# kfirc1503/generative-audio

Measured on AMD Instinct MI355X. Metric: spectrogram-frames/sec, NPPC K=5 FullSubNet+ train step, higher is better.
Workload: dtype bf16

## Files before the change

generative-audio_amd/csrc/tcn.hip:

```cpp
#include <cstdlib>
#include "common.h"
#include "nppc_hip.h"

namespace {

enum { EPI_PLAIN = 0, EPI_PRELU_STATS = 1, EPI_RESIDUAL = 2, EPI_RELU = 3, EPI_PLAIN_F32 = 4, EPI_MASK_POS = 5, EPI_RESIDUAL_GN = 6 };

struct GemmArgs {
  const void* A; long lda; long strideA;
  const void* B; long ldb; long strideB;
  void* C; long ldc; long strideC;
  const float* bias; long strideBias;
  const void* res; long ldres; long strideRes;
  const float* slope; long strideSlope;
  double* stats; long strideStats;
  int R, N, K;
  int Tp, Tv;
  int Nv;
  int relu_in;
  int ksplit;
  const float* gnv; long strideGnv;
  double gcnt; float geps;
  int staged;
  float* colpart; long strideColpart;
// ... 1190 lines not shown
  dma_tile<DR_BM, BN, BR, STAGES>(A, lda, B, ldb, C + (size_t)bz * slab_stride, ldc, (long)bx * DR_BM, (long)by * BN, (long)by * BN,
                           rbase + (shift_a ? boff : 0), rbase + (shift_a ? 0 : boff), Rz, rs);
}

template <int BM, int BR, int STAGES>
__global__ __launch_bounds__(512, 1) void gemm_tn_dma2_kernel(const bf16_t* __restrict__ A, long lda, const bf16_t* __restrict__ B1,
                                                              long ldb1, int nt1, const bf16_t* __restrict__ B2, long ldb2, int N2,
                                                              float* __restrict__ C, long ldc, long slab_stride, long Rz,
                                                              float* __restrict__ rowsum) {
  unsigned bx = blockIdx.x, by = blockIdx.y, bz = blockIdx.z;
  dr_xcd_remap(bx, by, bz);
  const long m0 = (long)bx * BM, rbase = (long)bz * Rz;
  float* Cz = C + (size_t)bz * slab_stride;
  float* rs = rowsum != nullptr && by == 0 ? rowsum + (size_t)bz * ((size_t)gridDim.x * BM) : nullptr;
  if ((int)by >= nt1 && N2 == 64) {
    dma_tile<BM, 64, BR, STAGES>(A, lda, B2, ldb2, Cz, ldc, m0, 0, (long)nt1 * 192, rbase, rbase, Rz, nullptr);
    return;
  }
  const bool second = (int)by >= nt1;
  const long n0 = (long)(second ? by - nt1 : by) * 192;
  dma_tile<BM, 192, BR, STAGES>(A, lda, second ? B2 : B1, second ? ldb2 : ldb1, Cz, ldc, m0, n0, (long)by * 192, rbase, rbase, Rz, rs);
}

}

static bool tn_big_tiles() {
  static int v = -1;
  if (v < 0) {
    const char* e = getenv("NPPC_TN_BIG");
    v = (e && e[0] == '0') ? 0 : 1;
  }
  return v == 1;
}

static bool tn_dma() {
  static int v = -1;
  if (v < 0) {
    const char* e = getenv("NPPC_TN_DMA");
    v = (e && e[0] == '0') ? 0 : 1;
  }
  return v == 1;
}

static bool tn_dma192() {
  static int v = -1;
  if (v < 0) {
// ... 92 lines not shown
    return NPPC_OK;
  }
  if (M % DR_BM || (long)(M / DR_BM) * (nt1 + nt2) * ksplit < 256) return NPPC_EUNSUPPORTED;
  constexpr int smem = 5 * (32 * DR_BM * 2 + 32 * 192 * 2);
  static bool attr = false;
  if (!attr) {
    if (hipFuncSetAttribute(reinterpret_cast<const void*>(gemm_tn_dma2_kernel<DR_BM, 32, 5>),
                            hipFuncAttributeMaxDynamicSharedMemorySize, smem) != hipSuccess)
      return NPPC_ELAUNCH;
    attr = true;
  }
  hipLaunchKernelGGL((gemm_tn_dma2_kernel<DR_BM, 32, 5>), dim3(M / DR_BM, nt1 + nt2, ksplit), dim3(512), smem, s, (const bf16_t*)A,
                     lda, (const bf16_t*)B1, ldb1, nt1, (const bf16_t*)B2, ldb2, N2, C, ldc, (long)M * ldc, R / ksplit, rowsum);
  NPPC_CHECK_LAUNCH();
  return NPPC_OK;
}

extern "C" int nppc_gemm_tn_splitk_batched(const void* A, long lda, long sA, const void* B, long ldb, long sB, float* C, long ldc,
                                           long sC, int M, int N, long R, int ksplit, int batch, void* stream) {
  if (batch < 1) return NPPC_EBADARG;
  return launch_tn(A, lda, B, ldb, C, ldc, M, N, R, ksplit, 1, 0, 0, stream, batch, sA, sB, sC);
}

extern "C" int nppc_gemm_tn_splitk_taps(const void* A, long lda, const void* B, long ldb, float* C, long ldc, int M, int N,
                                        long R, int ksplit, int Wp, int shift_a, void* stream) {
  return launch_tn(A, lda, B, ldb, C, ldc, M, N, R, ksplit, 9, Wp, shift_a, stream);
}
```

generative-audio_amd/csrc/train_ops.hip:

```cpp
#include "common.h"
#include "nppc_hip.h"

namespace {

template <typename T>
__global__ __launch_bounds__(256) void transpose_kernel(const T* __restrict__ in, T* __restrict__ out, int rows, int cols,
                                                        long ld_in, long ld_out, long sIn, long sOut, int relu) {
  __shared__ float tile[32][33];
  in += (size_t)blockIdx.z * sIn;
  out += (size_t)blockIdx.z * sOut;
  const int r0 = blockIdx.x * 32, c0 = blockIdx.y * 32;
  const int tx = threadIdx.x & 31, ty = threadIdx.x >> 5;
  for (int i = ty; i < 32; i += 8) {
    const int r = r0 + i, c = c0 + tx;
    float v = 0.f;
    if (r < rows && c < cols) v = to_f32<T>(in[(size_t)r * ld_in + c]);
    if (relu) v = fmaxf(v, 0.f);
    tile[i][tx] = v;
  }
  __syncthreads();
  for (int i = ty; i < 32; i += 8) {
    const int c = c0 + i, r = r0 + tx;
    if (c < cols && r < rows) out[(size_t)c * ld_out + r] = from_f32<T>(tile[tx][i]);
  }
// ... 318 lines not shown
    float* d = dst + (size_t)rr * dst_ld + c;
    *d = accumulate ? *d + s : s;
  }
}

__global__ void reduce_slabs_t_kernel(const float* __restrict__ slabs, int S, long slab_stride, long ld, float* __restrict__ dst,
                                      long dst_ld, int rows, int ncols, long sSlab, long sDst) {
  slabs += (size_t)blockIdx.z * sSlab;
  dst += (size_t)blockIdx.z * sDst;
  __shared__ float tile[32][33];
  const int c0 = blockIdx.x * 32, r0 = blockIdx.y * 32;
  const int tx = threadIdx.x & 31, ty = threadIdx.x >> 5;
  for (int i = ty; i < 32; i += 8) {
    const int c = c0 + i, r = r0 + tx;
    float a = 0.f;
    if (c < ncols && r < rows)
      for (int s = 0; s < S; ++s) a += slabs[(size_t)s * slab_stride + (size_t)c * ld + r];
    tile[i][tx] = a;
  }
  __syncthreads();
  for (int i = ty; i < 32; i += 8) {
    const int r = r0 + i, c = c0 + tx;
    if (r < rows && c < ncols) dst[(size_t)r * dst_ld + c] = tile[tx][i];
  }
}

__global__ void adam_kernel(float* __restrict__ p, const float* __restrict__ g, float* __restrict__ m, float* __restrict__ v,
                            long n, float lr, float b1, float b2, float eps, float wd, float bc1, float bc2_sqrt,
                            float gscale, const double* __restrict__ sumsq, float max_norm,
                            const unsigned* const* __restrict__ guards = nullptr, int n_guards = 0, float* poison = nullptr) {
  for (int i = 0; i < n_guards; ++i)
    if (*guards[i] != 0u) {
      if (poison && blockIdx.x == 0 && threadIdx.x == 0) *poison = __builtin_nanf("");
      return;
    }
  if (sumsq) {
    const float total = (float)sqrt(sumsq[0]) * gscale;
    const float coef = max_norm / (total + 1e-6f);
    gscale *= coef < 1.f ? coef : 1.f;
  }
  for (long i = (long)blockIdx.x * blockDim.x + threadIdx.x; i < n; i += (long)gridDim.x * blockDim.x) {
    float gi = g[i] * gscale;
    const float pi = p[i];
    if (wd != 0.f) gi += wd * pi;
    const float mi = b1 * m[i] + (1.f - b1) * gi;
    const float vi = b2 * v[i] + (1.f - b2) * gi * gi;
// ... 167 lines not shown
  return NPPC_OK;
}

int nppc_reduce_slabs(const float* slabs, int S, long slab_stride, long ld, float* dst, long dst_ld, int rows, int col0,
                      int ncols, int permH, int accumulate, long sSlab, long sDst, int batch, void* stream) {
  if (!slabs || !dst || S < 1 || rows <= 0 || ncols <= 0) return NPPC_EBADARG;
  const long total = (long)rows * ncols;
  const int gx = (int)((total + 255) / 256 > 1024 ? 1024 : (total + 255) / 256);
  hipLaunchKernelGGL(reduce_slabs_kernel, dim3(gx, 1, batch), dim3(256), 0, (hipStream_t)stream, slabs, S, slab_stride, ld,
                     dst, dst_ld, rows, col0, ncols, permH, accumulate, sSlab, sDst);
  NPPC_CHECK_LAUNCH();
  return NPPC_OK;
}

int nppc_reduce_slabs_t(const float* slabs, int S, long slab_stride, long ld, float* dst, long dst_ld, int rows, int ncols,
                        long sSlab, long sDst, int batch, void* stream) {
  if (!slabs || !dst || S < 1 || rows <= 0 || ncols <= 0 || batch < 1) return NPPC_EBADARG;
  hipLaunchKernelGGL(reduce_slabs_t_kernel, dim3(ceil_div(ncols, 32), ceil_div(rows, 32), batch), dim3(256), 0,
                     (hipStream_t)stream, slabs, S, slab_stride, ld, dst, dst_ld, rows, ncols, sSlab, sDst);
  NPPC_CHECK_LAUNCH();
  return NPPC_OK;
}

int nppc_adam_step(float* p, const float* g, float* m, float* v, long n, double lr, double b1, double b2, double eps,
                   double wd, int step, double gscale, void* stream) {
  if (!p || !g || !m || !v || n <= 0 || step < 1) return NPPC_EBADARG;
  const double bc1 = 1.0 - pow(b1, (double)step);
  const double bc2s = sqrt(1.0 - pow(b2, (double)step));
  const int grid = (int)((n + 255) / 256 > 2048 ? 2048 : (n + 255) / 256);
  hipLaunchKernelGGL(adam_kernel, dim3(grid), dim3(256), 0, (hipStream_t)stream, p, g, m, v, n, (float)lr, (float)b1, (float)b2,
                     (float)eps, (float)wd, (float)bc1, (float)bc2s, (float)gscale, (const double*)nullptr, 0.f);
  NPPC_CHECK_LAUNCH();
  return NPPC_OK;
}

int nppc_adam_step_guarded(float* p, const float* g, float* m, float* v, long n, double lr, double b1, double b2, double eps,
                           double wd, int step, double gscale, const void* guards, int n_guards, float* poison, void* stream) {
  if (!p || !g || !m || !v || n <= 0 || step < 1 || n_guards < 0 || (n_guards > 0 && !guards)) return NPPC_EBADARG;
  const double bc1 = 1.0 - pow(b1, (double)step);
  const double bc2s = sqrt(1.0 - pow(b2, (double)step));
  const int grid = (int)((n + 255) / 256 > 2048 ? 2048 : (n + 255) / 256);
  hipLaunchKernelGGL(adam_kernel, dim3(grid), dim3(256), 0, (hipStream_t)stream, p, g, m, v, n, (float)lr, (float)b1, (float)b2,
                     (float)eps, (float)wd, (float)bc1, (float)bc2s, (float)gscale, (const double*)nullptr, 0.f,
                     (const unsigned* const*)guards, n_guards, poison);
  NPPC_CHECK_LAUNCH();
  return NPPC_OK;
// ... 16 lines not shown
```

generative-audio_amd/nppc_audio/_hip.py:

```python
import ctypes
import os

import torch

_HERE = os.path.dirname(os.path.abspath(__file__))
LIB_PATH = os.environ.get("NPPC_HIP_LIB") or os.path.join(_HERE, "libnppc_hip.so")

PREC_BF16 = 0
PREC_F32 = 1
_ERR = {1: "bad argument", 2: "kernel launch failed", 3: "unsupported shape/configuration"}

_lib = None

c_p = ctypes.c_void_p
c_i = ctypes.c_int
c_l = ctypes.c_long
c_f = ctypes.c_float


def lib():
    global _lib
    if _lib is None:
        if not os.path.exists(LIB_PATH):
            raise RuntimeError(
# ... 95 lines not shown
    "nppc_cirm_build_compress": [P, P, P, P, P, I, I, I, I, F, P],
    "nppc_cirm_decompress_apply_conj": [P, P, P, P, P, P, P, I, I, I, P],
    "nppc_cirm_decompress_apply": [P, P, P, P, P, P, P, I, I, I, P],
    "nppc_istft": [P, P, P, I, I, I, I, I, P],
    "nppc_rowsum": [P, P, L, I, P],
    "nppc_tsse_fwd": [P, P, P, P, P, P, P, P, I, I, I, P, P, P, P, P, P, P, P, P, P, P, P, I, I, I, I, P],
    "nppc_tsse_fwd_maps": [I, P, I, P, P, P, P, P, P, P, I, I, I, P, P, P, P, P, P, L, P, P, P, P, P, P, P, L, I, I, I, I, I, I, P],
    "nppc_tsse_bwd_maps": [I, P, L, P, I, P, P, P, P, I, I, I, P, P, P, L, P, P, P, P, P, P, P, P, P, P, P, P, P, P, P, P, P, P,
                           I, I, I, I, I, I, P],
    "nppc_scale_transpose": [I, P, P, P, I, I, I, I, I, I, P],
    "nppc_gemm_nt": [I, I, P, L, L, P, L, L, P, L, L, P, L, P, L, L, P, L, P, L, I, I, I, I, I, I, I, I, I, P],
    "nppc_tcn_mid_bwd_part_elems": [I, I, I, I, PL],
    "nppc_tcn_mid_bwd": [I, P, P, P, P, P, P, P, P, P, P, P, P, P, P, P, P, P, P, P, P, P, P, P, P, P, P, I, I, I, P,
                         I, I, I, I, I, F, L, L, L, I, I, P],
    "nppc_tcn_mid_bwd_finish": [P, L, P, L, I, I, I, P, P, P, P, P, P, P, P, P, P, I, I, L, L, I, I, P],
    "nppc_gemm_nt_colsum": [I, I, P, L, L, P, L, L, P, L, L, P, L, P, L, L, I, I, I, I, I, I, I, P, P],
    "nppc_gemm_nt_gn": [I, P, L, L, P, L, L, P, L, L, P, P, L, P, L, L, P, L, D, F, I, I, I, I, I, I, I, P],
    "nppc_tcn_pack_sconv": [I, P, P, P, P, P, P, P, I, I, I, I, I, I, L, L, L, L, P],
    "nppc_gemm_nt_splitk": [I, P, L, P, L, P, L, I, I, L, I, P],
    "nppc_gemm_tn_splitk": [P, L, P, L, P, L, I, I, L, I, P],
    "nppc_gemm_tn_splitk_rowsum": [P, L, P, L, P, L, I, I, L, I, P, P],
    "nppc_gemm_tn_splitk2": [P, L, P, L, I, P, L, I, P, L, I, L, I, P, P],
    "nppc_gemm_tn_splitk_batched": [P, L, L, P, L, L, P, L, L, I, I, L, I, I, P],
    "nppc_reduce_slabs_t": [P, I, L, L, P, L, I, I, L, L, I, P],
    "nppc_gemm_tn_splitk_taps": [P, L, P, L, P, L, I, I, L, I, I, I, P],
    "nppc_tcn_dwconv": [I, P, P, P, P, P, P, P, P, P, I, I, I, I, I, I, F, L, L, L, I, P],
    "nppc_tcn_gn_apply": [I, P, P, P, P, P, I, I, I, I, I, F, L, L, L, I, P],
    "nppc_pack_matrix": [I, P, P, I, I, I, I, I, P],
    "nppc_pack_matrix_batched": [I, P, P, I, I, I, I, I, I, I, L, L, L, L, P],
    "nppc_subband_mean": [I, P, I, P, I, L, P, P, P, I, I, I, I, I, P],
    "nppc_subband_stage": [I, P, I, P, I, L, P, P, I, I, I, I, I, I, I, I, P],
    "nppc_sb_head": [I, P, P, P, P, L, I, I, I, I, I, P],
    "nppc_gram": [P, P, P, P, P, I, I, L, P],
    "nppc_combine": [P, P, P, P, P, P, P, I, I, L, P],
    "nppc_gs_solve": [P, P, P, I, I, I, P],
    "nppc_gs_bwd_solve": [P, P, P, P, I, I, I, P],
    "nppc_loss_solve": [P, P, P, P, P, P, P, P, P, P, I, I, P],
    "nppc_loss_bwd_coef": [P, P, P, F, F, P, I, I, P],
    "nppc_loss_bwd_coef_dev": [P, P, P, P, F, F, P, I, I, P],
    "nppc_transpose": [I, P, P, I, I, L, L, L, L, I, I, P],
    "nppc_colsum": [I, P, P, I, I, L, L, L, I, P, L, P],
    "nppc_colsum_scratch_elems": [I, I, I, PL],
    "nppc_sb_head_bwd": [I, P, P, P, P, P, P, L, I, I, I, I, I, P],
    "nppc_subband_stage_bwd": [I, P, P, P, P, P, P, I, I, I, I, I, L, I, I, I, P],
    "nppc_subband_unfold_bwd": [I, P, P, P, P, P, I, I, I, I, I, I, I, I, P],
    "nppc_reduce_slabs": [P, I, L, L, P, L, I, I, I, I, I, L, L, I, P],
# ... 146 lines not shown
```

generative-audio_amd/nppc_audio/engine.py:

```python
import ctypes
import os

import numpy as np
import torch

from . import _hip as H
from .ops_lstm import (PackedLSTM, PackedLSTMBwd, ROW_PAD, WGRAD_SPLITS, bwd_head_fusable, forward_x_ld, lstm2_backward, lstm2_forward,
                       own_workspaces, padded_rows,
                       rows_view, workspace)

TCN_HIDDEN = 512
TCN_DILATIONS = (1, 2, 5, 9, 1, 2, 5, 9)
BRANCHES = ("", "_real", "_imag")
EPI_PLAIN, EPI_PRELU_STATS, EPI_RESIDUAL, EPI_RELU, EPI_PLAIN_F32, EPI_MASK_POS = 0, 1, 2, 3, 4, 5


def rup(a, b):
    return (a + b - 1) // b * b


TCN_WGRAD_ON_SIDE = os.environ.get("NPPC_TCN_WGRAD_SIDE", "1") != "0"
TCN_WGRAD_SPLITS = int(os.environ.get("NPPC_TCN_S2", "8"))
FC_WGRAD_AT_END = os.environ.get("NPPC_FC_AT_END", "1") != "0"
TCN_WGRAD_MAIN_BLOCKS = int(os.environ.get("NPPC_TCN_WGRAD_MAIN_BLOCKS", "1"))
MID_FINISH_DEFER = os.environ.get("NPPC_MID_FINISH_DEFER", "1") != "0"
COLSUM_IN_GEMM = os.environ.get("NPPC_COLSUM_IN_GEMM", "1") != "0"
TN_PAIRED = os.environ.get("NPPC_TN_PAIRED", "1") != "0"
FUSED_HEAD = int(os.environ.get("NPPC_FUSED_HEAD", "3"))


class FlatParams:

    def __init__(self, module, device):
        named = list(module.named_parameters())
        total = sum(p.numel() for _, p in named)
        self.flat = torch.empty(total, dtype=torch.float32, device=device)
        self.grad = None
        self.off = {}
        o = 0
        for n, p in named:
            k = p.numel()
            self.flat[o:o + k].copy_(p.detach().reshape(-1))
            p.data = self.flat[o:o + k].view(p.shape)
            self.off[n] = (o, tuple(p.shape))
            o += k
        self.named = named

    def view(self, name):
        o, shp = self.off[name]
# ... 49 lines not shown

class FSNEngine:
    import weakref as _weakref
    _unjoined = _weakref.WeakValueDictionary()

    def __init__(self, flat, *, num_freqs, n_maps, out_size, sb_neighbors, look_ahead, sb_hidden, groups, kersize,
                 prec, trainable):
        self.fp = flat
        self.F, self.nm, self.O = num_freqs, n_maps, out_size
        self.nb, self.la, self.Hd, self.G = sb_neighbors, look_ahead, sb_hidden, groups
        self.ks = tuple(kersize)
        self.prec = prec
        self.dt = H.dtype_of(prec)
        self.trainable = trainable
        self.C = n_maps * num_freqs
        self.ldC = rup(self.C, 64)
        self.ldF = rup(num_freqs, 64)
        self.KC = self.ldC
        self.dev = flat.flat.device
        self.I = 2 * sb_neighbors + 1 + 3
        self.sP = flat.branch_stride()
        self.sAtt = flat.attention_stride()
        self.packed_version = None
        self._side = None
        self._gen = 0
        self.last_train = None
        self.grad_range_hook = None
        self.early_buckets_ok = self._check_bucket_layout() if trainable else False
        self.pre_lstm_hook = None
        self.defer_join = False
        self.join_pending = False
        self.bufs = {}
        own_workspaces(self)
        self.lstm = PackedLSTM(self.I, self.Hd, prec, self.dev)
        self.KX = self.lstm.kx
        self.mult = torch.from_numpy(unfold_multiplicity(self.F, self.nb)).to(self.dev)
        C, ldC, ldF = self.C, self.ldC, self.ldF
        self.W1p = torch.zeros(8, 3, TCN_HIDDEN, ldC, dtype=self.dt, device=self.dev)
        self.W2p = torch.zeros(8, 3, ldC, TCN_HIDDEN, dtype=self.dt, device=self.dev)
        self.u2 = torch.zeros(8, 3, ldC, dtype=torch.float32, device=self.dev)
        self.v2 = torch.zeros(8, 3, ldC, dtype=torch.float32, device=self.dev)
        self.Wfcp = torch.zeros(3, ldF, ldC, dtype=self.dt, device=self.dev)
        self.Opad = rup(self.O, 16)
        self.Whp = torch.zeros(self.Opad, self.Hd, dtype=self.dt, device=self.dev)
        if trainable:
            if self.O > 32:
# ... 403 lines not shown
            with torch.cuda.stream(self._side):
                self._side.wait_event(ev)
                fn()

        def fc_wgrad(slab):
            q = H.stream()
            H.colsum(prec, dpre_fb, self.g("fb_model.fc_output_layer.bias"), R, F, ldF, R * ldF, sP, 3,
                     lambda n: ws("cs_fc", (n,), torch.float32), q)
            H.call("nppc_transpose", prec, dpre_fb, tA, R, F, ldF, R, R * ldF, sTA, 0, 3, q)
            H.call("nppc_transpose", prec, X8, tB, R, ldC, ldC, R, R * ldC, sTB, 1, 3, q)
            self._wgrad(tA, R, sTA, tB, R, sTB, Fr, ldC, R, S2, "fb_model.fc_output_layer.weight", C, F, C, slab, batch=3, sDst=sP)
        fc_ok = prec == H.PREC_BF16 and TCN_HIDDEN % 128 == 0 and ldC % 64 == 0 and R % (64 * S2) == 0
        fc_at_end = fc_ok and FC_WGRAD_AT_END
        if fc_ok and not fc_at_end:
            on_side(lambda: fc_wgrad(slab2))
        elif not fc_ok:
            fc_wgrad(slab2)
        tn_ok = prec == H.PREC_BF16 and TCN_HIDDEN % 128 == 0 and ldC % 64 == 0 and R % (64 * S2) == 0
        if tn_ok:
            dXL = [ws(f"dX_{i}", (3, B, Tp, ldC)) for i in range(9)]
            a2L = [ws(f"a2_{i}", (3, B, Tp, TCN_HIDDEN), zero=True) for i in range(8)]
            h2L = [ws(f"h2b_{i}", (3, B, Tp, TCN_HIDDEN)) for i in range(8)]
            dXa, dXb = dXL[8], dXL[7]
        else:
            dXa = ws("dXa", (3, B, Tp, ldC))
            dXb = ws("dXb", (3, B, Tp, ldC))

        bk = 64 if prec == H.PREC_BF16 else 32
        cs_ok = tn_ok and COLSUM_IN_GEMM and ldF % bk == 0 and TCN_HIDDEN % bk == 0
        cp_all = ws("colpart", (8, 3, R // 128, ldC), torch.float32) if cs_ok else None
        cpL = [cp_all[i] for i in range(8)] if cs_ok else None
        if cs_ok:
            H.call("nppc_gemm_nt_colsum", prec, EPI_MASK_POS, dpre_fb, ldF, R * ldF, self.WfcT, ldF, ldC * ldF, dXa, ldC, R * ldC,
                   None, 0, X8, ldC, R * ldC, R, ldC, ldF, Tp, Tv, C, 3, cpL[7], s)
        else:
            H.call("nppc_gemm_nt", prec, EPI_MASK_POS, dpre_fb, ldF, R * ldF, self.WfcT, ldF, ldC * ldF, dXa, ldC, R * ldC, None, 0,
                   X8, ldC, R * ldC, None, 0, None, 0, R, ldC, ldF, Tp, Tv, C, 0, 3, 1, s)
        sAct = B * Tp * TCN_HIDDEN
        h1b = ws("h1b", (3, B, Tp, TCN_HIDDEN))
        h2b = ws("h2b", (3, B, Tp, TCN_HIDDEN))
        Smid = ws("Smid", (3, B, TCN_HIDDEN // 64, 8), torch.float64)
        n_part = H.mid_bwd_part_elems(B, TCN_HIDDEN, Tp, 3)
        Pmid = ws("Pmid", (8, n_part), torch.float32)
        lay = self.fp.off["fb_model.sequence_model.1.conv1x1.weight"][0] - self.fp.off["fb_model.sequence_model.0.conv1x1.weight"][0]

        def finish_mid(lo, hi):
            pre_ = f"fb_model.sequence_model.{lo}."
            H.call("nppc_tcn_mid_bwd_finish", Pmid[lo], n_part, cpL[lo] if cs_ok else None, 3 * (R // 128) * ldC, R // 128, ldC, C,
                   self.g(pre_ + "norm2.weight"), self.g(pre_ + "norm2.bias"), self.g(pre_ + "norm1.weight"), self.g(pre_ + "norm1.bias"),
                   self.g(pre_ + "depthwise_conv.weight"), self.g(pre_ + "depthwise_conv.bias"), self.g(pre_ + "prelu1.weight"),
                   self.g(pre_ + "prelu2.weight"), self.g(pre_ + "conv1x1.bias"), self.g(pre_ + "sconv.bias") if cs_ok else None,
                   B, TCN_HIDDEN, sP, lay, 3, hi - lo, s)
        early = self.grad_range_hook is not None and self.early_buckets_ok
        defer_finish = MID_FINISH_DEFER
        dXo, dXi = dXa, dXb
        for i in range(7, -1, -1):
            pre = f"fb_model.sequence_model.{i}."
            dil = TCN_DILATIONS[i]
            st1, st2 = d["stats"][i, 0], d["stats"][i, 1]
            y1, y2, Xin = d["y1"][i], d["y2"][i], d["X"][i]
            if tn_ok:
                dXo, dXi, a2, h2b = dXL[i + 1], dXL[i], a2L[i], h2L[i]
            else:
                a2 = d["a2"]
            if not cs_ok:
                H.colsum(prec, dXo, self.g(pre + "sconv.bias"), R, C, ldC, R * ldC, sP, 3,
                         lambda n: ws("cs_sconv", (n,), torch.float32), s)
            H.call("nppc_gemm_nt", prec, EPI_PLAIN, dXo, ldC, R * ldC, self.W2T[i], ldC, TCN_HIDDEN * ldC, h1b, TCN_HIDDEN,
                   sAct, None, 0, None, 0, 0, None, 0, None, 0, R, TCN_HIDDEN, ldC, Tp, Tv, TCN_HIDDEN, 0, 3, 1, s)
            H.call("nppc_tcn_mid_bwd", prec, h1b, y2, y1, st1, st2, Smid, Pmid[i], self.p(pre + "norm1.weight"), self.p(pre + "norm1.bias"),
                   self.p(pre + "norm2.weight"), self.p(pre + "norm2.bias"), self.p(pre + "depthwise_conv.weight"),
                   self.p(pre + "prelu1.weight"), self.p(pre + "prelu2.weight"), a2, h2b, self.g(pre + "norm2.weight"),
                   self.g(pre + "norm2.bias"), self.g(pre + "norm1.weight"), self.g(pre + "norm1.bias"),
                   self.g(pre + "depthwise_conv.weight"), self.g(pre + "depthwise_conv.bias"), self.g(pre + "prelu1.weight"),
                   self.g(pre + "prelu2.weight"), self.g(pre + "conv1x1.bias"),
                   cpL[i] if cs_ok else None, R // 128, ldC, C, self.g(pre + "sconv.bias") if cs_ok else None,
                   B, TCN_HIDDEN, Tp, Tv, dil, 1e-8, sAct, B * 2, sP, 3, 0 if defer_finish else 1, s)
            if i == 4 and early and defer_finish:
                finish_mid(4, 8)
            if tn_ok:
                inline = i < TCN_WGRAD_MAIN_BLOCKS
                wslab = ws("slab_main", (3 * S2 * TCN_HIDDEN * ldC,), torch.float32) if inline else slab2

                def sconv_wgrad(a2=a2, dXo=dXo, dest=self.g(pre + "sconv.weight"), wslab=wslab):
                    q = H.stream()
                    H.call("nppc_gemm_tn_splitk_batched", a2, TCN_HIDDEN, sAct, dXo, ldC, R * ldC, wslab, ldC,
                           S2 * TCN_HIDDEN * ldC, TCN_HIDDEN, ldC, R, S2, 3, q)
                    H.call("nppc_reduce_slabs_t", wslab, S2, TCN_HIDDEN * ldC, ldC, dest, TCN_HIDDEN, C, TCN_HIDDEN,
                           S2 * TCN_HIDDEN * ldC, sP, 3, q)
                if inline:
                    sconv_wgrad()
                else:
                    on_side(sconv_wgrad)
            else:
                H.call("nppc_transpose", prec, dXo, tA, R, ldC, ldC, R, R * ldC, sTA, 0, 3, s)
                H.call("nppc_transpose", prec, a2, tB, R, TCN_HIDDEN, TCN_HIDDEN, R, sAct, sTB, 0, 3, s)
                self._wgrad(tA, R, sTA, tB, R, sTB, Cr, TCN_HIDDEN, R, S2, pre + "sconv.weight", TCN_HIDDEN, C, TCN_HIDDEN,
                            slab2, batch=3, sDst=sP)
            if tn_ok:
                def c1_wgrad(h2b=h2b, Xin=Xin, dest=self.g(pre + "conv1x1.weight"), wslab=wslab):
                    q = H.stream()
                    H.call("nppc_gemm_tn_splitk_batched", h2b, TCN_HIDDEN, sAct, Xin, ldC, R * ldC, wslab, ldC,
                           S2 * TCN_HIDDEN * ldC, TCN_HIDDEN, ldC, R, S2, 3, q)
                    H.call("nppc_reduce_slabs", wslab, S2, TCN_HIDDEN * ldC, ldC, dest, C, TCN_HIDDEN, 0, C, 0, 0,
                           S2 * TCN_HIDDEN * ldC, sP, 3, q)
                if inline:
                    c1_wgrad()
                else:
                    on_side(c1_wgrad)
            else:
                H.call("nppc_transpose", prec, h2b, tA, R, TCN_HIDDEN, TCN_HIDDEN, R, sAct, sTA, 0, 3, s)
                H.call("nppc_transpose", prec, Xin, tB, R, ldC, ldC, R, R * ldC, sTB, 0, 3, s)
                self._wgrad(tA, R, sTA, tB, R, sTB, TCN_HIDDEN, ldC, R, S2, pre + "conv1x1.weight", C, TCN_HIDDEN, C, slab2,
                            batch=3, sDst=sP)
            if cs_ok and i > 0:
                H.call("nppc_gemm_nt_colsum", prec, EPI_RESIDUAL, h2b, TCN_HIDDEN, sAct, self.W1T[i], TCN_HIDDEN, ldC * TCN_HIDDEN,
                       dXi, ldC, R * ldC, None, 0, dXo, ldC, R * ldC, R, ldC, TCN_HIDDEN, Tp, Tv, C, 3, cpL[i - 1], s)
            else:
                H.call("nppc_gemm_nt", prec, EPI_RESIDUAL, h2b, TCN_HIDDEN, sAct, self.W1T[i], TCN_HIDDEN, ldC * TCN_HIDDEN, dXi, ldC,
                       R * ldC, None, 0, dXo, ldC, R * ldC, None, 0, None, 0, R, ldC, TCN_HIDDEN, Tp, Tv, C, 0, 3, 1, s)
            dXo, dXi = dXi, dXo
            if i == 4 and self.grad_range_hook is not None and self.early_buckets_ok:
# ... 60 lines not shown
```

include/nppc_hip.h:

```cpp
#ifndef NPPC_HIP_H
#define NPPC_HIP_H
#ifdef __cplusplus
extern "C" {
#endif

int nppc_stft(const float* wave, float* re, float* im, float* mag , int B, int L, int nfft, int hop,
              void* stream);
int nppc_dropband(const float* in, float* out, int B, int C, int F, int T, int G, void* stream);
int nppc_cirm_build_compress(const float* nr, const float* ni, const float* cr, const float* ci, float* out, int B, int F,
                             int T, int G, float eps, void* stream);
int nppc_cirm_decompress_apply_conj(const float* crm, const float* nr, const float* ni, float* dec ,
                                    float* emag, float* ere, float* eim, int B, int F, int T, void* stream);

int nppc_cirm_decompress_apply(const float* crm, const float* nr, const float* ni, float* dec , float* emag,
                               float* ere, float* eim, int B, int F, int T, void* stream);
int nppc_istft(const float* re, const float* im, float* out, int B, int T, int nfft, int hop, int L, void* stream);

int nppc_rowsum(const float* x, double* sums, long R, int T, void* stream);
int nppc_tsse_fwd_maps(int prec, const float* const* maps, int nmaps, double* rowsum, const float* cw0, const float* cb0,
                       const float* cw1, const float* cb1, const float* cw2, const float* cb2, int ks0, int ks1, int ks2,
                       const float* fcw, const float* fcb, const float* w1, const float* b1, const float* w2, const float* b2, long sW,
                       float* scale, float* ns, float* pre, float* sq, float* h1, float* sg, void* X0, long sY, int B, int C, int T,
                       int look_ahead, int Tp, int ld, void* stream);
int nppc_tsse_bwd_ws_elems(int nmaps, int B, int C, int ks0, int ks1, int ks2, long* elems);
// ... 11 lines not shown
int nppc_tsse_bwd(int prec, const void* dX0, const float* x, const double* rowsum, const float* cw0, const float* cw1,
                  const float* cw2, int ks0, int ks1, int ks2, const float* fcw, const float* w1, const float* w2,
                  const float* ns, const float* pre, const float* sq, const float* h1, const float* sg, float* dsg_ws,
                  float* g_cw0, float* g_cb0, float* g_cw1, float* g_cb1, float* g_cw2, float* g_cb2, float* g_fcw,
                  float* g_fcb, float* g_w1, float* g_b1, float* g_w2, float* g_b2, int B, int C, int T, int look_ahead, int Tp,
                  int ld, int coff, void* stream);
int nppc_scale_transpose(int prec, const float* x, const float* scale , void* y, int B, int C, int T, int Tp,
                         int ld, int coff, void* stream);

int nppc_gemm_nt(int prec, int epi, const void* A, long lda, long sA, const void* B, long ldb, long sB, void* C, long ldc,
                 long sC, const float* bias, long sBias, const void* res, long ldres, long sRes, const float* slope,
                 long sSlope, double* stats, long sStats, int R, int N, int K, int Tp, int Tv, int Nv, int relu_in,
                 int batch, int ksplit, void* stream);
int nppc_gemm_nt_splitk(int prec, const void* A, long lda, const void* B, long ldb, float* C, long ldc, int M, int N, long K,
                        int ksplit, void* stream);
int nppc_gemm_tn_splitk(const void* A, long lda, const void* B, long ldb, float* C, long ldc, int M, int N, long R, int ksplit,
                        void* stream);
int nppc_gemm_tn_splitk_rowsum(const void* A, long lda, const void* B, long ldb, float* C, long ldc, int M, int N, long R,
                               int ksplit, float* rowsum, void* stream);
int nppc_gemm_tn_splitk2(const void* A, long lda, const void* B1, long ldb1, int N1, const void* B2, long ldb2, int N2, float* C,
                         long ldc, int M, long R, int ksplit, float* rowsum, void* stream);
int nppc_gemm_tn_splitk_batched(const void* A, long lda, long sA, const void* B, long ldb, long sB, float* C, long ldc, long sC,
                                int M, int N, long R, int ksplit, int batch, void* stream);
int nppc_gemm_tn_splitk_taps(const void* A, long lda, const void* B, long ldb, float* C, long ldc, int M, int N, long R,
                             int ksplit, int Wp, int shift_a, void* stream);
int nppc_pack_matrix(int prec, const float* src, void* dst, int N, int K, int Npad, int ldd, int transpose, void* stream);
int nppc_pack_matrix_batched(int prec, const float* src, void* dst, int N, int K, int Npad, int ldd, int transpose, int n_a,
                             int n_b, long src_stride_a, long src_stride_b, long dst_stride_a, long dst_stride_b, void* stream);
int nppc_tcn_dwconv(int prec, const void* in, void* out, const double* st1, double* st2, const float* gamma,
                    const float* beta, const float* wd, const float* bd, const float* slope2, int B, int Cc, int ld, int Tp,
                    int Tv, int dil, float eps, long sAct, long sSt, long sP, int batch, void* stream);
int nppc_tcn_gn_apply(int prec, const void* in, void* out, const double* st, const float* gamma, const float* beta, int B,
                      int Cc, int ld, int Tp, int Tv, float eps, long sAct, long sSt, long sP, int batch, void* stream);
int nppc_tcn_gn_bwd(int prec, const void* dA, const void* y, const double* st, const float* gamma, const float* slope,
                    double* S, void* dpre, float* dgamma, float* dbeta, float* dslope, int B, int Cc, int Tp, int Tv, float eps,
                    long sAct, long sSt, long sP, int batch, void* stream);
int nppc_tcn_dwconv_bwd(int prec, const void* du, const void* y1, const double* st1, const float* gamma, const float* beta,
                        const float* wd, void* dz, float* dwd, float* dbd, int B, int Cc, int Tp, int Tv, int dil, float eps,
                        long sAct, long sSt, long sP, int batch, void* stream);
int nppc_tcn_mid_bwd_part_elems(int B, int Cc, int Tp, int batch, long* n);
int nppc_tcn_mid_bwd(int prec, const void* dA, const void* y2, const void* y1, const double* st1, const double* st2, double* S,
                     float* part,
                     const float* gamma1, const float* beta1, const float* gamma2, const float* beta2, const float* wd,
                     const float* slope1, const float* slope2, void* a2, void* dpre1, float* dgamma2, float* dbeta2,
                     float* dgamma1, float* dbeta1, float* dwd, float* dbd, float* dslope1, float* dslope2, float* dbias1,
                     const float* colpart, int cp_tiles, int cp_ld, int cp_cols, float* dbias2, int B,
                     int Cc, int Tp, int Tv, int dil, float eps, long sAct, long sSt, long sP, int batch, int finish_now,
                     void* stream);
int nppc_tcn_mid_bwd_finish(const float* part, long partL, const float* colpart, long colpartL, int cp_tiles, int cp_ld,
                            int cp_cols, float* dgamma2, float* dbeta2, float* dgamma1, float* dbeta1, float* dwd, float* dbd,
                            float* dslope1, float* dslope2, float* dbias1, float* dbias2, int B, int Cc, long sP, long sL,
                            int batch, int nblk, void* stream);
int nppc_gemm_nt_gn(int prec, const void* A, long lda, long sA, const void* Wg, long ldb, long sB, void* C, long ldc, long sC,
                    const float* u, const float* v, long sUV, const void* res, long ldres, long sRes, const double* stats,
                    long sStats, double cnt, float eps, int R, int N, int K, int Tp, int Tv, int Nv, int batch, void* stream);
int nppc_gemm_nt_colsum(int prec, int epi, const void* A, long lda, long sA, const void* B, long ldb, long sB, void* C, long ldc,
                        long sC, const float* bias, long sBias, const void* res, long ldres, long sRes, int R, int N, int K,
                        int Tp, int Tv, int Nv, int batch, float* colpart, void* stream);
int nppc_tcn_pack_sconv(int prec, const float* W, const float* gamma, const float* beta, const float* bias, void* Wg, float* u,
                        float* v, int N, int K, int Npad, int ldd, int n_a, int n_b, long src_stride_a, long src_stride_b,
                        long dst_stride_a, long dst_stride_b, void* stream);
int nppc_transpose(int prec, const void* in, void* out, int rows, int cols, long ld_in, long ld_out, long sIn, long sOut,
                   int relu, int batch, void* stream);
int nppc_colsum_scratch_elems(int rows, int cols, int batch, long* n);
int nppc_colsum(int prec, const void* M, float* out, int rows, int cols, long ld, long sM, long sOut, int batch,
                float* scratch, long scratch_elems, void* stream);
int nppc_reduce_slabs_t(const float* slabs, int S, long slab_stride, long ld, float* dst, long dst_ld, int rows, int ncols,
                        long sSlab, long sDst, int batch, void* stream);
int nppc_reduce_slabs(const float* slabs, int S, long slab_stride, long ld, float* dst, long dst_ld, int rows, int col0,
                      int ncols, int permH, int accumulate, long sSlab, long sDst, int batch, void* stream);

int nppc_subband_mean(int prec, const void* src, int ldS, const void* fb, int ldF, long strideFb, const float* mult,
                      float* scale, double* work, int B, int F, int Tp, int Tv, int nfeat, void* stream);
int nppc_subband_stage(int prec, const void* src, int ldS, const void* fb, int ldF, long strideFb, const float* scale,
                       void* x, int B, int F, int Tp, int Tv, int nb, int G, int KX, int ones_col, void* stream);
int nppc_subband_stage_bwd(int prec, const void* dx, const void* x, const void* fb, const float* scale, double* D,
                           void* dpre, int B, int F, int Tp, int Tv, int ldF, long strideFb, int nb, int G, int KX,
                           void* stream);
int nppc_subband_unfold_bwd(int prec, const void* dx, const float* scale, const double* D, const float* mult, void* dX0,
                            int ldX, int B, int F, int Tp, int Tv, int nb, int G, int KX, void* stream);
int nppc_sb_head(int prec, const void* h2, const void* wh, const float* bias, float* out, long Nseq, int Tn, int la,
                 int Hd, int O, int Fo, void* stream);
int nppc_sb_head_bwd(int prec, const float* dout, const void* whT, const void* h2, void* dh2, float* dWh, float* dbh,
                     long Nseq, int Tn, int la, int Hd, int O, int Fo, void* stream);

int nppc_lstm2_packed_elems(int I, int H, long* n1, long* n2, int* kx);
int nppc_lstm2_pack_weights(int prec, const float* w_ih0, const float* w_hh0, const float* b_ih0, const float* b_hh0,
                            const float* w_ih1, const float* w_hh1, const float* b_ih1, const float* b_hh1, int I, int H,
                            void* wp1, void* wp2, float* bias1, float* bias2, void* stream);
int nppc_lstm2_fwd(int prec, int train, int mtile, const void* x, const void* wp1, const void* wp2, const float* bias1,
                   const float* bias2, void* h2, void* h1, void* g1, void* g2, void* c1, void* c2, long N, int Tn, int I,
// ... 336 lines not shown
```

Before: 254,900.

## Group TCN weight-gradient GEMMs across blocks into single grouped split-K launches

Adds a grouped TN split-K GEMM kernel that takes per-problem pointer tables, plus a grouped slab-reduction kernel that vectorises reads and can write either transposed or plain output. The engine accumulates the sconv and conv1x1 weight-gradient GEMMs of several TCN blocks and issues them as one grouped GEMM and one grouped reduce on the side stream. This replaces many small per-block launches and separate transposes, which should cut launch overhead and improve GPU fill. In exchange, gradients become available later for the groups, and the pointer tables are cached per set of data pointers.

```diff
diff --git a/generative-audio_amd/csrc/tcn.hip b/generative-audio_amd/csrc/tcn.hip
--- a/generative-audio_amd/csrc/tcn.hip
+++ b/generative-audio_amd/csrc/tcn.hip
@@ -1236,6 +1236,36 @@
   dma_tile<BM, 192, BR, STAGES>(A, lda, second ? B2 : B1, second ? ldb2 : ldb1, Cz, ldc, m0, n0, (long)by * 192, rbase, rbase, Rz, rs);
 }
 
+constexpr int TN_GROUP_MAX = 48;
+struct TnGroup {
+  const bf16_t* A[TN_GROUP_MAX];
+  const bf16_t* B[TN_GROUP_MAX];
+  float* C[TN_GROUP_MAX];
+  int lda[TN_GROUP_MAX], ldb[TN_GROUP_MAX], ldc[TN_GROUP_MAX];
+};
+
+__device__ __forceinline__ void dr_xcd_remap_any(unsigned& bx, unsigned& by, unsigned& bz) {
+  const unsigned tiles = gridDim.x * gridDim.y;
+  const unsigned lin = bx + gridDim.x * (by + gridDim.y * bz);
+  if (lin < tiles * (gridDim.z & ~7u)) {
+    const unsigned xcd = lin & 7, j = lin >> 3;
+    bz = xcd + 8 * (j / tiles);
+    const unsigned t = j % tiles;
+    bx = t % gridDim.x;
+    by = t / gridDim.x;
+  }
+}
+
+template <int BN, int BR, int STAGES>
+__global__ __launch_bounds__(512, 1) void gemm_tn_dma_grouped_kernel(const TnGroup g, int M, long Rz, int ksplit) {
+  unsigned bx = blockIdx.x, by = blockIdx.y, bz = blockIdx.z;
+  dr_xcd_remap_any(bx, by, bz);
+  const unsigned p = bz / (unsigned)ksplit, z = bz % (unsigned)ksplit;
+  const long ldc = g.ldc[p];
+  dma_tile<DR_BM, BN, BR, STAGES>(g.A[p], g.lda[p], g.B[p], g.ldb[p], g.C[p] + (size_t)z * M * ldc, ldc, (long)bx * DR_BM,
+                                  (long)by * BN, (long)by * BN, (long)z * Rz, (long)z * Rz, Rz, nullptr);
+}
+
 }
 
 static bool tn_big_tiles() {
@@ -1374,6 +1404,57 @@
   return launch_tn(A, lda, B, ldb, C, ldc, M, N, R, ksplit, 1, 0, 0, stream, batch, sA, sB, sC);
 }
 
+extern "C" int nppc_gemm_tn_grouped(const void* const* A, const long* lda, const void* const* B, const long* ldb, float* const* C,
+                                    const long* ldc, int M, int N, long R, int ksplit, int P, void* stream) {
+  if (!A || !lda || !B || !ldb || !C || !ldc || M <= 0 || N <= 0 || R <= 0 || ksplit < 1 || P < 1) return NPPC_EBADARG;
+  if (P > TN_GROUP_MAX || (long)P * ksplit > 65535 || !tn_dma() || M % DR_BM || R % ksplit) return NPPC_EUNSUPPORTED;
+  const int bn = N % 192 == 0 ? 192 : (N % 128 == 0 ? 128 : 0);
+  const long Rz = R / ksplit;
+  if (bn == 0 || Rz % (bn == 192 ? 32 : 64)) return NPPC_EUNSUPPORTED;
+  TnGroup g;
+  for (int p = 0; p < P; ++p) {
+    if (!A[p] || !B[p] || !C[p] || lda[p] < M || ldb[p] < N || ldc[p] < N || lda[p] % 8 || ldb[p] % 8) return NPPC_EBADARG;
+    if (lda[p] > 0x7fffffffL || ldb[p] > 0x7fffffffL || ldc[p] > 0x7fffffffL) return NPPC_EBADARG;
+    if (((size_t)A[p] | (size_t)B[p]) & 15) return NPPC_EBADARG;
+    g.A[p] = (const bf16_t*)A[p];
+    g.B[p] = (const bf16_t*)B[p];
+    g.C[p] = C[p];
+    g.lda[p] = (int)lda[p];
+    g.ldb[p] = (int)ldb[p];
+    g.ldc[p] = (int)ldc[p];
+  }
+  for (int p = P; p < TN_GROUP_MAX; ++p) {
+    g.A[p] = g.B[p] = nullptr;
+    g.C[p] = nullptr;
+    g.lda[p] = g.ldb[p] = g.ldc[p] = 0;
+  }
+  hipStream_t s = (hipStream_t)stream;
+  dim3 grid(M / DR_BM, N / bn, P * ksplit);
+  if (bn == 192) {
+    constexpr int smem = 5 * (32 * DR_BM * 2 + 32 * 192 * 2);
+    static bool attr = false;
+    if (!attr) {
+      if (hipFuncSetAttribute(reinterpret_cast<const void*>(gemm_tn_dma_grouped_kernel<192, 32, 5>),
+                              hipFuncAttributeMaxDynamicSharedMemorySize, smem) != hipSuccess)
+        return NPPC_ELAUNCH;
+      attr = true;
+    }
+    hipLaunchKernelGGL((gemm_tn_dma_grouped_kernel<192, 32, 5>), grid, dim3(512), smem, s, g, M, Rz, ksplit);
+  } else {
+    constexpr int smem = 3 * (64 * DR_BM * 2 + 64 * 128 * 2);
+    static bool attr = false;
+    if (!attr) {
+      if (hipFuncSetAttribute(reinterpret_cast<const void*>(gemm_tn_dma_grouped_kernel<128, 64, 3>),
+                              hipFuncAttributeMaxDynamicSharedMemorySize, smem) != hipSuccess)
+        return NPPC_ELAUNCH;
+      attr = true;
+    }
+    hipLaunchKernelGGL((gemm_tn_dma_grouped_kernel<128, 64, 3>), grid, dim3(512), smem, s, g, M, Rz, ksplit);
+  }
+  NPPC_CHECK_LAUNCH();
+  return NPPC_OK;
+}
+
 extern "C" int nppc_gemm_tn_splitk_taps(const void* A, long lda, const void* B, long ldb, float* C, long ldc, int M, int N,
                                         long R, int ksplit, int Wp, int shift_a, void* stream) {
   return launch_tn(A, lda, B, ldb, C, ldc, M, N, R, ksplit, 9, Wp, shift_a, stream);
diff --git a/generative-audio_amd/csrc/train_ops.hip b/generative-audio_amd/csrc/train_ops.hip
--- a/generative-audio_amd/csrc/train_ops.hip
+++ b/generative-audio_amd/csrc/train_ops.hip
@@ -364,6 +364,55 @@
   for (int i = ty; i < 32; i += 8) {
     const int r = r0 + i, c = c0 + tx;
     if (r < rows && c < ncols) dst[(size_t)r * dst_ld + c] = tile[tx][i];
+  }
+}
+
+constexpr int SLAB_GROUP_MAX = 48;
+struct SlabGroup {
+  const float* slab[SLAB_GROUP_MAX];
+  float* dst[SLAB_GROUP_MAX];
+  int dst_ld[SLAB_GROUP_MAX];
+  unsigned long long transposed;
+};
+
+__global__ __launch_bounds__(256) void reduce_slabs_grouped_kernel(const SlabGroup g, int S, long slab_stride, long ld, int rows,
+                                                                   int ncols) {
+  const unsigned p = blockIdx.z;
+  const float* __restrict__ slabs = g.slab[p];
+  float* __restrict__ dst = g.dst[p];
+  const long dst_ld = g.dst_ld[p];
+  const bool tr = (g.transposed >> p) & 1ull;
+  __shared__ float tile[32][33];
+  const int c0 = blockIdx.x * 32, r0 = blockIdx.y * 32;
+  const int q = threadIdx.x & 7, rr = threadIdx.x >> 3;
+  {
+    const int r = r0 + rr, c = c0 + 4 * q;
+    float4 a = make_float4(0.f, 0.f, 0.f, 0.f);
+    if (r < rows && c < ncols) {
+      const float* src = slabs + (size_t)r * ld + c;
+      for (int s = 0; s < S; ++s) {
+        const float4 v = *reinterpret_cast<const float4*>(src + (size_t)s * slab_stride);
+        a.x += v.x;
+        a.y += v.y;
+        a.z += v.z;
+        a.w += v.w;
+      }
+    }
+    tile[rr][4 * q + 0] = a.x;
+    tile[rr][4 * q + 1] = a.y;
+    tile[rr][4 * q + 2] = a.z;
+    tile[rr][4 * q + 3] = a.w;
+  }
+  __syncthreads();
+  const int tx = threadIdx.x & 31, ty = threadIdx.x >> 5;
+  for (int i = ty; i < 32; i += 8) {
+    if (tr) {
+      const int c = c0 + i, r = r0 + tx;
+      if (r < rows && c < ncols) dst[(size_t)c * dst_ld + r] = tile[tx][i];
+    } else {
+      const int r = r0 + i, c = c0 + tx;
+      if (r < rows && c < ncols) dst[(size_t)r * dst_ld + c] = tile[i][tx];
+    }
   }
 }
 
@@ -577,6 +626,32 @@
   return NPPC_OK;
 }
 
+int nppc_reduce_slabs_grouped(const float* const* slabs, float* const* dst, const long* dst_ld, const int* transposed, int P, int S,
+                              long slab_stride, long ld, int rows, int ncols, void* stream) {
+  if (!slabs || !dst || !dst_ld || !transposed || P < 1 || S < 1 || rows <= 0 || ncols <= 0 || ncols > ld) return NPPC_EBADARG;
+  if (ld % 4 || slab_stride % 4 || slab_stride < (long)rows * ld) return NPPC_EBADARG;
+  if (P > SLAB_GROUP_MAX) return NPPC_EUNSUPPORTED;
+  SlabGroup g;
+  g.transposed = 0ull;
+  for (int p = 0; p < SLAB_GROUP_MAX; ++p) {
+    g.slab[p] = nullptr;
+    g.dst[p] = nullptr;
+    g.dst_ld[p] = 0;
+  }
+  for (int p = 0; p < P; ++p) {
+    const long need = transposed[p] ? rows : ncols;
+    if (!slabs[p] || !dst[p] || ((size_t)slabs[p] & 15) || dst_ld[p] < need || dst_ld[p] > 0x7fffffffL) return NPPC_EBADARG;
+    g.slab[p] = slabs[p];
+    g.dst[p] = dst[p];
+    g.dst_ld[p] = (int)dst_ld[p];
+    if (transposed[p]) g.transposed |= 1ull << p;
+  }
+  hipLaunchKernelGGL(reduce_slabs_grouped_kernel, dim3(ceil_div(ncols, 32), ceil_div(rows, 32), P), dim3(256), 0,
+                     (hipStream_t)stream, g, S, slab_stride, ld, rows, ncols);
+  NPPC_CHECK_LAUNCH();
+  return NPPC_OK;
+}
+
 int nppc_adam_step(float* p, const float* g, float* m, float* v, long n, double lr, double b1, double b2, double eps,
                    double wd, int step, double gscale, void* stream) {
   if (!p || !g || !m || !v || n <= 0 || step < 1) return NPPC_EBADARG;
diff --git a/generative-audio_amd/nppc_audio/_hip.py b/generative-audio_amd/nppc_audio/_hip.py
--- a/generative-audio_amd/nppc_audio/_hip.py
+++ b/generative-audio_amd/nppc_audio/_hip.py
@@ -141,6 +141,8 @@
     "nppc_gemm_tn_splitk_rowsum": [P, L, P, L, P, L, I, I, L, I, P, P],
     "nppc_gemm_tn_splitk2": [P, L, P, L, I, P, L, I, P, L, I, L, I, P, P],
     "nppc_gemm_tn_splitk_batched": [P, L, L, P, L, L, P, L, L, I, I, L, I, I, P],
+    "nppc_gemm_tn_grouped": [P, P, P, P, P, P, I, I, L, I, I, P],
+    "nppc_reduce_slabs_grouped": [P, P, P, P, I, I, L, L, I, I, P],
     "nppc_reduce_slabs_t": [P, I, L, L, P, L, I, I, L, L, I, P],
     "nppc_gemm_tn_splitk_taps": [P, L, P, L, P, L, I, I, L, I, I, I, P],
     "nppc_tcn_dwconv": [I, P, P, P, P, P, P, P, P, P, I, I, I, I, I, I, F, L, L, L, I, P],
diff --git a/generative-audio_amd/nppc_audio/engine.py b/generative-audio_amd/nppc_audio/engine.py
--- a/generative-audio_amd/nppc_audio/engine.py
+++ b/generative-audio_amd/nppc_audio/engine.py
@@ -17,6 +17,12 @@
 
 def rup(a, b):
     return (a + b - 1) // b * b
+
+
+def tn_grouped_supported(M, N, R, S):
+    if M % 256 or S < 1 or R % S:
+        return False
+    return (N % 192 == 0 and (R // S) % 32 == 0) or (N % 192 != 0 and N % 128 == 0 and (R // S) % 64 == 0)
 
 
 TCN_WGRAD_ON_SIDE = os.environ.get("NPPC_TCN_WGRAD_SIDE", "1") != "0"
@@ -25,6 +31,9 @@
 TCN_WGRAD_MAIN_BLOCKS = int(os.environ.get("NPPC_TCN_WGRAD_MAIN_BLOCKS", "1"))
 MID_FINISH_DEFER = os.environ.get("NPPC_MID_FINISH_DEFER", "1") != "0"
 COLSUM_IN_GEMM = os.environ.get("NPPC_COLSUM_IN_GEMM", "1") != "0"
+TCN_WGRAD_GROUPED = os.environ.get("NPPC_TCN_WGRAD_GROUPED", "1") != "0"
+TCN_WGRAD_GROUP_BLOCKS = int(os.environ.get("NPPC_TCN_WGRAD_GROUP_BLOCKS", "4"))
+TCN_WGRAD_GROUP_SPLITS = int(os.environ.get("NPPC_TCN_WGRAD_GROUP_S", "8"))
 TN_PAIRED = os.environ.get("NPPC_TN_PAIRED", "1") != "0"
 FUSED_HEAD = int(os.environ.get("NPPC_FUSED_HEAD", "3"))
 
@@ -120,6 +129,7 @@
         self.sP = flat.branch_stride()
         self.sAtt = flat.attention_stride()
         self.packed_version = None
+        self._grp_tabs = {}
         self._side = None
         self._gen = 0
         self.last_train = None
@@ -569,7 +579,10 @@
             a2L = [ws(f"a2_{i}", (3, B, Tp, TCN_HIDDEN), zero=True) for i in range(8)]
             h2L = [ws(f"h2b_{i}", (3, B, Tp, TCN_HIDDEN)) for i in range(8)]
             dXa, dXb = dXL[8], dXL[7]
-        else:
+            Sg = TCN_WGRAD_GROUP_SPLITS if R % (64 * TCN_WGRAD_GROUP_SPLITS) == 0 else S2
+            grouped = TCN_WGRAD_GROUPED and tn_grouped_supported(TCN_HIDDEN, ldC, R, Sg)
+        else:
+            grouped = False
             dXa = ws("dXa", (3, B, Tp, ldC))
             dXb = ws("dXb", (3, B, Tp, ldC))
 
@@ -598,7 +611,39 @@
                    self.g(pre_ + "depthwise_conv.weight"), self.g(pre_ + "depthwise_conv.bias"), self.g(pre_ + "prelu1.weight"),
                    self.g(pre_ + "prelu2.weight"), self.g(pre_ + "conv1x1.bias"), self.g(pre_ + "sconv.bias") if cs_ok else None,
                    B, TCN_HIDDEN, sP, lay, 3, hi - lo, s)
+        pending = []
+
+        def issue_group(items, tag):
+            n = 3 * len(items)
+            slab_e = TCN_HIDDEN * ldC
+            slab = ws(f"slab_grp_{tag}", (n * Sg * slab_e,), torch.float32)
+            key = (slab.data_ptr(), Sg) + tuple((a.data_ptr(), b.data_ptr(), g_.data_ptr(), t) for a, b, g_, t in items)
+            tabs = self._grp_tabs.get(key)
+            if tabs is None:
+                vp, lg = ctypes.c_void_p * n, ctypes.c_long * n
+                Ap, Bp, Cp, Dp, dl, tr = [], [], [], [], [], []
+                for j, (a, b, g_, t) in enumerate(items):
+                    for z in range(3):
+                        Ap.append(a.data_ptr() + z * sAct * a.element_size())
+                        Bp.append(b.data_ptr() + z * R * ldC * b.element_size())
+                        Cp.append(slab.data_ptr() + (3 * j + z) * Sg * slab_e * 4)
+                        Dp.append(g_.data_ptr() + z * sP * 4)
+                        dl.append(TCN_HIDDEN if t else C)
+                        tr.append(1 if t else 0)
+                tabs = (vp(*Ap), lg(*([TCN_HIDDEN] * n)), vp(*Bp), lg(*([ldC] * n)), vp(*Cp), lg(*([ldC] * n)), vp(*Dp), lg(*dl),
+                        (ctypes.c_int * n)(*tr))
+                self._grp_tabs[key] = tabs
+            Aa, la, Ba, lb, Ca, lc, Da, dla, tra = tabs
+
+            def run():
+                q = H.stream()
+                H.call("nppc_gemm_tn_grouped", Aa, la, Ba, lb, Ca, lc, TCN_HIDDEN, ldC, R, Sg, n, q)
+                H.call("nppc_reduce_slabs_grouped", Ca, Da, dla, tra, n, Sg, slab_e, ldC, TCN_HIDDEN, C, q)
+            on_side(run)
         early = self.grad_range_hook is not None and self.early_buckets_ok
+        gblocks = min(TCN_WGRAD_GROUP_BLOCKS, 4) if early else TCN_WGRAD_GROUP_BLOCKS
+        if gblocks not in (1, 2, 4, 8):
+            raise ValueError(f"NPPC_TCN_WGRAD_GROUP_BLOCKS must be 1, 2, 4 or 8, not {TCN_WGRAD_GROUP_BLOCKS}")
         defer_finish = MID_FINISH_DEFER
         dXo, dXi = dXa, dXb
         for i in range(7, -1, -1):
@@ -625,7 +670,13 @@
                    B, TCN_HIDDEN, Tp, Tv, dil, 1e-8, sAct, B * 2, sP, 3, 0 if defer_finish else 1, s)
             if i == 4 and early and defer_finish:
                 finish_mid(4, 8)
-            if tn_ok:
+            if grouped:
+                pending.append((a2, dXo, self.g(pre + "sconv.weight"), True))
+                pending.append((h2b, Xin, self.g(pre + "conv1x1.weight"), False))
+                if i % gblocks == 0:
+                    issue_group(pending, f"{i + gblocks - 1}_{i}")
+                    pending = []
+            elif tn_ok:
                 inline = i < TCN_WGRAD_MAIN_BLOCKS
                 wslab = ws("slab_main", (3 * S2 * TCN_HIDDEN * ldC,), torch.float32) if inline else slab2
 
@@ -644,7 +695,9 @@
                 H.call("nppc_transpose", prec, a2, tB, R, TCN_HIDDEN, TCN_HIDDEN, R, sAct, sTB, 0, 3, s)
                 self._wgrad(tA, R, sTA, tB, R, sTB, Cr, TCN_HIDDEN, R, S2, pre + "sconv.weight", TCN_HIDDEN, C, TCN_HIDDEN,
                             slab2, batch=3, sDst=sP)
-            if tn_ok:
+            if grouped:
+                pass
+            elif tn_ok:
                 def c1_wgrad(h2b=h2b, Xin=Xin, dest=self.g(pre + "conv1x1.weight"), wslab=wslab):
                     q = H.stream()
                     H.call("nppc_gemm_tn_splitk_batched", h2b, TCN_HIDDEN, sAct, Xin, ldC, R * ldC, wslab, ldC,
diff --git a/include/nppc_hip.h b/include/nppc_hip.h
--- a/include/nppc_hip.h
+++ b/include/nppc_hip.h
@@ -57,6 +57,8 @@
                          long ldc, int M, long R, int ksplit, float* rowsum, void* stream);
 int nppc_gemm_tn_splitk_batched(const void* A, long lda, long sA, const void* B, long ldb, long sB, float* C, long ldc, long sC,
                                 int M, int N, long R, int ksplit, int batch, void* stream);
+int nppc_gemm_tn_grouped(const void* const* A, const long* lda, const void* const* B, const long* ldb, float* const* C,
+                         const long* ldc, int M, int N, long R, int ksplit, int P, void* stream);
 int nppc_gemm_tn_splitk_taps(const void* A, long lda, const void* B, long ldb, float* C, long ldc, int M, int N, long R,
                              int ksplit, int Wp, int shift_a, void* stream);
 int nppc_pack_matrix(int prec, const float* src, void* dst, int N, int K, int Npad, int ldd, int transpose, void* stream);
@@ -102,6 +104,8 @@
                 float* scratch, long scratch_elems, void* stream);
 int nppc_reduce_slabs_t(const float* slabs, int S, long slab_stride, long ld, float* dst, long dst_ld, int rows, int ncols,
                         long sSlab, long sDst, int batch, void* stream);
+int nppc_reduce_slabs_grouped(const float* const* slabs, float* const* dst, const long* dst_ld, const int* transposed, int P, int S,
+                              long slab_stride, long ld, int rows, int ncols, void* stream);
 int nppc_reduce_slabs(const float* slabs, int S, long slab_stride, long ld, float* dst, long dst_ld, int rows, int col0,
                       int ncols, int permH, int accumulate, long sSlab, long sDst, int batch, void* stream);
 
```

After: 255,100 (median of 2 runs). About the same (+0.1%).
